# UZ-SLAMLab/DefSLAM

Measured on AMD Instinct MI355X. Metric: SfT GN iters/sec (500-node mesh, 1k matches), higher is better.
Workload: dtype f64

## Files before the change

defslam_amd/csrc/sft_batch.h:

```cpp
#pragma once

#define SFTB_NW 8
#ifndef SFTB_LIN_NW
#define SFTB_LIN_NW 8
#endif
#ifndef SFTB_LIN_WAVES
#define SFTB_LIN_WAVES 2
#endif
#ifndef SFTB_TRIAL_WAVES
#define SFTB_TRIAL_WAVES 2
#endif

__device__ __forceinline__ void sftb_ctl_lds(char* smem, Ctl*& ctl, double*& red, double*& out, double*& panel) {
  ctl = reinterpret_cast<Ctl*>(smem);
  red = reinterpret_cast<double*>(smem + 512);
  out = red + 16 * 27 + 5;
  panel = out + 32;
}

__global__ __launch_bounds__(64 * SFTB_NW, 2) void sftb_init_kernel(const SftDev* __restrict__ probs, SftRun* __restrict__ runs, int* __restrict__ counters, int* __restrict__ lin_list, int tail_below) {
  const SftDev& P = probs[blockIdx.x];
  if (blockIdx.x == 0 && threadIdx.x == 0 && (int)gridDim.x <= tail_below) counters[6] = 1;
  init_state<64 * SFTB_NW>(P);
  if (threadIdx.x == 0) {
    SftRun& R = runs[blockIdx.x];
    R.lambda = -1.0; R.ni = 2.0; R.chi_cur = 0.0; R.chi_ini = 0.0; R.rho = 0.0; R.lambda_start = 0.0;
    R.it = 0; R.qmax = 0; R.nbad = 0; R.accepted = 0; R.all_ok = 1; R.iters = 0; R.trials = 0; R.fact_ok = 1;
    R.state = P.max_iters > 0 ? SFTB_LIN : SFTB_FINISH;
    if (P.max_iters > 0) lin_list[atomicAdd(&counters[2], 1)] = blockIdx.x;
  }
}

template <int NW>
__device__ __forceinline__ void sftb_lin_problem(const SftDev& P, SftRun& R, Ctl* ctl, double* red, double* out, double* panel) {
  constexpr int NT = 64 * NW;
  const int tid = threadIdx.x;
  auto nothing = [] {};
  const double chi0 = linearise<NW, decltype(nothing), true>(P, ctl, red, out, panel, nothing);
  double lambda = R.lambda;
  if (R.it == 0) {
    double mx = 0.0;
    for (int r = tid; r < P.Dn; r += NT) mx = fmax(mx, fabs(h_diag(P, r)));
    if (tid < 6) mx = fmax(mx, fabs(P.Hcorner[tid * 8]));
    mx = block_max(mx, red);
    lambda = 1e-5 * mx;
  }
  if (tid == 0) {
    if (R.it == 0) { R.lambda = lambda; R.ni = 2.0; R.nbad = 0; }
    R.chi_cur = chi0; R.chi_ini = chi0; R.qmax = 0; R.rho = 0.0; R.accepted = 0; R.all_ok = 1; R.lambda_start = lambda;
    R.state = SFTB_TRIAL;
  }
}

__global__ __launch_bounds__(64 * SFTB_LIN_NW, SFTB_LIN_WAVES) void sftb_lin_kernel(const SftDev* __restrict__ probs, SftRun* __restrict__ runs, int* __restrict__ counters,
                                                                                  const int* __restrict__ lin_list, int B, int tail_below) {
  constexpr int NW = SFTB_LIN_NW, NT = 64 * NW;
  extern __shared__ __attribute__((aligned(16))) char smem[];
  __shared__ int next_b;
  Ctl* ctl; double *red, *out, *panel;
  sftb_ctl_lds(smem, ctl, red, out, panel);
  const int tid = threadIdx.x;
  if (counters[6] || B - counters[0] <= tail_below) {
    if (blockIdx.x == 0 && tid == 0) counters[6] = 1;
    return;
  }
  if (blockIdx.x == 0 && tid == 0) counters[7]++;
  auto fetch = [&]() { const int i = atomicAdd(&counters[3], 1); return i < counters[2] ? lin_list[i] : -1; };
  int nxt = -1;
  if (tid == 0) nxt = fetch();
  while (true) {
    if (tid == 0) next_b = nxt;
    __syncthreads();
    const int b = __builtin_amdgcn_readfirstlane(next_b);
    if (b < 0) break;
    if (tid == 0) { nxt = fetch(); atomicAdd(&counters[9], 1); }
    sftb_lin_problem<NW>(probs[b], runs[b], ctl, red, out, panel);
  }
}

__global__ __launch_bounds__(64, 1) void sftb_factor_kernel(const SftDev* __restrict__ probs, SftRun* __restrict__ runs, int* __restrict__ counters, int B) {
  extern __shared__ __attribute__((aligned(16))) char smem[];
  lds_double* lds = to_lds(reinterpret_cast<double*>(smem));
  const int lane = threadIdx.x;
  if (counters[6]) return;
  for (int i = lane; i < WV_LDS_DOUBLES; i += 64) lds[i] = 0.0;
  if (blockIdx.x == 0 && lane == 0) { counters[2] = 0; counters[3] = 0; }
  WvPrev Q;
  Q.Lg = nullptr; Q.Linv = nullptr; Q.x = nullptr; Q.nT = 0; Q.active = 0; Q.xb = 0.0;
  int n_done = 0;
  while (true) {
    int b = 0;
    if (lane == 0) b = atomicAdd(&counters[1], 1);
    b = __builtin_amdgcn_readfirstlane(b);
    if (b >= B) break;
    if (runs[b].state != SFTB_TRIAL) continue;
    const SftDev& P = probs[b];
    const double lambda = runs[b].lambda;
    double xcam;
    const int ok = wv_factor(P, lambda, lambda, lds, Q, xcam);
    if (lane == 0) runs[b].fact_ok = ok;
    Q = wv_prev_of(P, ok, xcam, lane);
    n_done++;
  }
  int lane_now;
  asm volatile("v_mbcnt_lo_u32_b32 %0, -1, 0\n\tv_mbcnt_hi_u32_b32 %0, -1, %0" : "=v"(lane_now));
  if (Q.active) wv_backsub_now(Q, lane_now);
  if (lane_now == 0 && n_done) atomicAdd(&counters[8], n_done);
}

template <int NW>
__device__ __forceinline__ int sftb_trial_problem(const SftDev& P, SftRun& R, Ctl* ctl, double* red, double* out, double* panel, int* counters, int* lin_list, int b) {
  constexpr int NT = 64 * NW;
  const int tid = threadIdx.x;
  const int Dn = P.Dn;
  const int Dnp = ((Dn + NB - 1) / NB) * NB;
  const int ok = R.fact_ok;
  const double lam = R.lambda;
  const bool in_lds = P.lds_class >= 1;
  if (!in_lds)
    for (int i = tid; i < 3 * P.n; i += NT) {
      const double v = P.xyz[i];
      P.xyz_bak[i] = v;
      const int a = P.act[i / 3];
      if (a >= 0) P.xyz[i] = v + P.x[3 * a + (i % 3)];
    }
  if (tid < 7) R.pose_bak[tid] = P.pose[tid];
  __syncthreads();
  if (tid == 0) pose_oplus(P.pose, P.x + Dnp);
  double sc = 0.0;
  for (int r = tid; r < Dn; r += NT) { const double xv = P.x[r]; sc += xv * (lam * xv + P.Hbord[(size_t)6 * Dnp + r]); }
  if (tid < 6) { const double xv = P.x[Dnp + tid]; sc += xv * (lam * xv + P.Hcorner[42 + tid]); }
  __syncthreads();
  block_sum<1>(&sc, red, out);
  const double scale = out[0];
  __syncthreads();
  const auto staged = asm_records<NW, 1>(P, panel);
  const double chi_new = in_lds ? eval_edges<false, 1>(P, ctl, red, out, staged, P.x)
                                : eval_edges<false, 0>(P, ctl, red, out, asm_records<NW, 0>(P, panel));
  if (tid == 0) {
    const double tempChi = ok ? chi_new : DBL_MAX;
    double rho = (R.chi_cur - tempChi);
    rho /= (scale + 1e-3);
    R.rho = rho;
    if (rho > 0 && isfinite(tempChi)) {
      double alpha = 1. - pow((2 * rho - 1), 3);
      alpha = fmin(alpha, 2. / 3.);
      const double sf = fmax(1. / 3., alpha);
      R.lambda = lam * sf; R.ni = 2.0; R.chi_cur = tempChi; R.accepted = 1;
      ctl->stop = 0;
    } else {
      R.lambda = lam * R.ni; R.ni *= 2.0;
      ctl->stop = 1;
    }
    R.qmax++;
    R.all_ok &= ok;
    ctl->qmax = R.qmax;
    ctl->rho = rho;
  }
  __syncthreads();
  if (ctl->stop) {
    if (!in_lds)
      for (int i = tid; i < 3 * P.n; i += NT) P.xyz[i] = P.xyz_bak[i];
    if (tid < 7) P.pose[tid] = R.pose_bak[tid];
  } else if (in_lds) {
    for (int i = tid; i < 3 * P.n; i += NT) P.xyz[i] = staged.xyz_l[i];
  }
  const bool again = (ctl->rho < 0) && (ctl->qmax < 10);
  if (again) return 0;
  __syncthreads();
  if (tid == 0) {
    const int qmax = R.qmax;
    R.trials += qmax;
    R.iters++;
    if (P.trace) {
      double* t = P.trace + R.it * 8;
      t[0] = R.chi_ini; t[1] = R.lambda_start; t[2] = qmax; t[3] = R.chi_cur; t[4] = R.lambda; t[5] = R.rho; t[6] = R.accepted; t[7] = R.all_ok;
    }
    if (!R.all_ok) P.res->status |= 1;
    bool term = (qmax == 10) || (R.rho == 0);
    if (!term) {
      if ((R.chi_ini - R.chi_cur) * 1e3 < R.chi_ini) R.nbad++; else R.nbad = 0;
      term = R.nbad >= 3;
    }
    R.it++;
    if (R.it >= P.max_iters) term = true;
    ctl->nbad = term ? 1 : 0;
    ctl->it = R.iters;
    ctl->accepted = R.trials;
    R.state = term ? SFTB_DONE : SFTB_LIN;
// ... 83 lines not shown
```

defslam_amd/csrc/sft_wave.h:

```cpp
#pragma once

#if defined(WV_STEP_TRACE) && defined(DSH_LAB)
#define WV_T_DECL long long wv_tr[9] = {0, 0, 0, 0, 0, 0, 0, 0, 0}, wv_tl = clock64()
#define WV_T(e) do { const long long t__ = clock64(); wv_tr[e] += t__ - wv_tl; wv_tl = t__; } while (0)
#define WV_T_ARG , long long (&wv_tr)[9], long long& wv_tl
#define WV_T_PASS , wv_tr, wv_tl
#define WV_T_DUMP(P) do { if ((threadIdx.x & 63) == 0) for (int e__ = 0; e__ < 9; e__++) (P).dbg[40 + e__] = (double)wv_tr[e__]; } while (0)
#else
#define WV_T_DECL do {} while (0)
#define WV_T(e) do {} while (0)
#define WV_T_ARG
#define WV_T_PASS
#define WV_T_DUMP(P) do {} while (0)
#endif

__host__ __device__ constexpr int wv_phys(int r, int d) {
  return d == 0 ? r : (d <= 3 ? 8 * d + r : (d == 4 ? 32 + (r & 3) : 8 * (8 - d) + ((r + 8 - d) & 7)));
}
constexpr int WV_AGPR_TILES = 32;
constexpr int WV_L_WIN = 0;
constexpr int WV_L_BORD = 1024;
constexpr int WV_L_WSCR = 2048;
constexpr int WV_L_CN = 2336;
constexpr int WV_L_XRING = 2400;
constexpr int WV_L_LAND = 2528;
constexpr int WV_LDS_DOUBLES = WV_L_LAND + 10 * 256;
typedef double v2d_w __attribute__((ext_vector_type(2)));
#ifndef WV_DMA_AUX
#define WV_DMA_AUX 0
#endif
using lds_v2d = __attribute__((address_space(3))) v2d_w;

#define WV_NOP_MFMA_RESULT "s_nop 15\n\ts_nop 3"

template <int T>
__device__ __forceinline__ void wv_upd_agpr(const v4d& A, const v4d& B, int q0 = 0) {
  static_assert(T >= 0 && T < WV_AGPR_TILES, "accumulator tile");
#define WV_MF(q) asm volatile("v_mfma_f64_16x16x4_f64 a[%c0:%c1], %2, %3, a[%c0:%c1] neg:[1,0,0]" ::"i"(8 * T), "i"(8 * T + 7), "v"(A[q]), "v"(B[q]) : "memory")
  if (q0 <= 0) WV_MF(0);
  if (q0 <= 1) WV_MF(1);
  if (q0 <= 2) WV_MF(2);
  WV_MF(3);
#undef WV_MF
}
__device__ __forceinline__ void wv_upd_vgpr(v4d& C, const v4d& A, const v4d& B, int q0 = 0) {
#define WV_MF(q) asm volatile("v_mfma_f64_16x16x4_f64 %0, %1, %2, %0 neg:[1,0,0]" : "+v"(C) : "v"(A[q]), "v"(B[q]) : "memory")
  asm volatile("s_nop 1" : "+v"(C));
  if (q0 <= 0) WV_MF(0);
  if (q0 <= 1) WV_MF(1);
  if (q0 <= 2) WV_MF(2);
  WV_MF(3);
#undef WV_MF
}
template <int T>
__device__ __forceinline__ void wv_trsm_agpr(v4d& Y, const v4d& Wt) {
  asm volatile("v_mfma_f64_16x16x4_f64 %0, %1, a[%c5:%c6], 0\n\t"
               "v_mfma_f64_16x16x4_f64 %0, %2, a[%c7:%c8], %0\n\t"
               "v_mfma_f64_16x16x4_f64 %0, %3, a[%c9:%c10], %0\n\t"
               "v_mfma_f64_16x16x4_f64 %0, %4, a[%c11:%c12], %0"
               : "=&v"(Y)
               : "v"(Wt[0]), "v"(Wt[1]), "v"(Wt[2]), "v"(Wt[3]), "i"(8 * T), "i"(8 * T + 1), "i"(8 * T + 2), "i"(8 * T + 3), "i"(8 * T + 4), "i"(8 * T + 5),
                 "i"(8 * T + 6), "i"(8 * T + 7)
               : "memory");
}
__device__ __forceinline__ void wv_trsm_vgpr(v4d& Y, const v4d& Wt, const v4d& D, int q0 = 0) {
  if (q0 <= 0) {
    asm volatile("s_nop 1\n\t"
                 "v_mfma_f64_16x16x4_f64 %0, %1, %5, 0\n\t"
                 "v_mfma_f64_16x16x4_f64 %0, %2, %6, %0\n\t"
                 "v_mfma_f64_16x16x4_f64 %0, %3, %7, %0\n\t"
                 "v_mfma_f64_16x16x4_f64 %0, %4, %8, %0"
                 : "=&v"(Y)
                 : "v"(Wt[0]), "v"(Wt[1]), "v"(Wt[2]), "v"(Wt[3]), "v"(D[0]), "v"(D[1]), "v"(D[2]), "v"(D[3])
                 : "memory");
  } else {
    asm volatile("s_nop 1\n\tv_mfma_f64_16x16x4_f64 %0, %1, %2, 0" : "=&v"(Y) : "v"(Wt[3]), "v"(D[3]) : "memory");
    if (q0 <= 2) asm volatile("v_mfma_f64_16x16x4_f64 %0, %1, %2, %0" : "+v"(Y) : "v"(Wt[2]), "v"(D[2]) : "memory");
    if (q0 <= 1) asm volatile("v_mfma_f64_16x16x4_f64 %0, %1, %2, %0" : "+v"(Y) : "v"(Wt[1]), "v"(D[1]) : "memory");
  }
}
struct WvTri { double a[10]; };
__device__ __forceinline__ void wv_tri_load(const lds_double* wscr, int lane, WvTri& A) {
  const lds_double* p = wscr + (lane & 3) * 17 + (lane >> 4);
#pragma unroll
  for (int q = 0; q < 4; q++)
#pragma unroll
    for (int k = 0; k <= q; k++) A.a[q * (q + 1) / 2 + k] = p[68 * q + 4 * k];
}
#define WV_TRI_BODY(D0, D1, D2, D3)                          \
  "v_mfma_f64_4x4x4_4b_f64 %3, %10, " D0 ", 0\n\t"   \
  "v_mfma_f64_4x4x4_4b_f64 %2, %7, " D0 ", 0\n\t"    \
  "v_mfma_f64_4x4x4_4b_f64 %3, %11, " D1 ", %3\n\t"  \
  "v_mfma_f64_4x4x4_4b_f64 %2, %8, " D1 ", %2\n\t"   \
  "v_mfma_f64_4x4x4_4b_f64 %3, %12, " D2 ", %3\n\t"  \
  "v_mfma_f64_4x4x4_4b_f64 %2, %9, " D2 ", %2\n\t"   \
  "v_mfma_f64_4x4x4_4b_f64 %3, %13, " D3 ", %3\n\t"  \
  "v_mfma_f64_4x4x4_4b_f64 %1, %5, " D0 ", 0\n\t"    \
  "v_mfma_f64_4x4x4_4b_f64 %0, %4, " D0 ", 0\n\t"    \
  "v_mfma_f64_4x4x4_4b_f64 %1, %6, " D1 ", %1"
template <int T>
__device__ __forceinline__ void wv_trsm4_agpr(v4d& Y, const WvTri& A) {
  asm volatile(WV_TRI_BODY("a[%c14:%c15]", "a[%c16:%c17]", "a[%c18:%c19]", "a[%c20:%c21]")
               : "=&v"(Y[0]), "=&v"(Y[1]), "=&v"(Y[2]), "=&v"(Y[3])
               : "v"(A.a[0]), "v"(A.a[1]), "v"(A.a[2]), "v"(A.a[3]), "v"(A.a[4]), "v"(A.a[5]), "v"(A.a[6]), "v"(A.a[7]), "v"(A.a[8]), "v"(A.a[9]),
                 "i"(8 * T), "i"(8 * T + 1), "i"(8 * T + 2), "i"(8 * T + 3), "i"(8 * T + 4), "i"(8 * T + 5), "i"(8 * T + 6), "i"(8 * T + 7)
               : "memory");
// ... 115 lines not shown
  w = (v4d){(g == c) ? 1.0 : 0.0, (g + 4 == c) ? 1.0 : 0.0, (g + 8 == c) ? 1.0 : 0.0, (g + 12 == c) ? 1.0 : 0.0};
  double plast = 1.0;
#pragma unroll
  for (int J = 0; J < 4; J++) {
    const double aJ = a[J];
    const double sel = chol4_inverse_operand(aJ, J, g, c & 3, plast);
    const double wJ = w[J];
    double zw, lp;
    if (J < 3) {
      asm volatile("s_nop 1\n\t"
                   "v_mfma_f64_4x4x4_4b_f64 %0, %2, %3, 0\n\t"
                   "v_mfma_f64_4x4x4_4b_f64 %1, %2, %4, 0\n\t"
                   "s_nop 7"
                   : "=&v"(zw), "=&v"(lp)
                   : "v"(sel), "v"(wJ), "v"(aJ));
      const double nlp = -lp;
      const double below = (c >= 4 * J + 4) ? nlp : 0.0;
      asm volatile("s_nop 1\n\t"
                   "v_mfma_f64_16x16x4_f64 %0, %2, %3, %0\n\t"
                   "v_mfma_f64_16x16x4_f64 %1, %4, %5, %1\n\t" WV_NOP_MFMA_RESULT
                   : "+v"(a), "+v"(w)
                   : "v"(nlp), "v"(lp), "v"(below), "v"(zw));
      w[J] = zw;
    } else {
      asm volatile("s_nop 1\n\tv_mfma_f64_4x4x4_4b_f64 %0, %1, %2, 0\n\ts_nop 7" : "=&v"(zw) : "v"(sel), "v"(wJ));
      w[J] = zw;
    }
  }
  return plast > 0.0;
}

struct WvProb {
  int Dn, Dnp, nT, q8;
  double lambda, lam_corner;
  unsigned bofs;
  const SFT_G double* Hc;
  const SFT_G uint32_t* hgl;
  const SFT_G double* Hbord;
  SFT_G double *Lg, *Linv;
};

typedef unsigned v4u_w __attribute__((ext_vector_type(4)));
__device__ __forceinline__ void wv_list(const WvProb& W, int I, int d, int lane, unsigned (&o)[4]) {
  const SFT_G v4u_w* row = reinterpret_cast<const SFT_G v4u_w*>(W.hgl + ((size_t)(I < W.nT ? I : W.nT) * (BT + 1) + d) * 256);
  const v4u_w v = row[lane];
  o[0] = v.x; o[1] = v.y; o[2] = v.z; o[3] = v.w;
}
__device__ __forceinline__ v4d wv_gather_vgpr(const WvProb& W, const unsigned (&o)[4]) {
  const auto b8 = reinterpret_cast<const SFT_G char*>(W.Hc);
  v4d v;
#pragma unroll
  for (int q = 0; q < 4; q++) v[q] = *reinterpret_cast<const SFT_G double*>(b8 + o[q]);
  return v;
}
__device__ __forceinline__ WvB2 wv_border_fresh(const WvProb& W, int J, int lane) {
  const SFT_G double* p = W.Hbord + TS * (J < W.nT ? J : W.nT);
  (void)lane;
  return WvB2{p[W.bofs], p[W.bofs + 4 * (unsigned)W.Dnp]};
}

struct WvRowList { unsigned o[8][4]; };
__device__ __forceinline__ void wv_row_list(const WvProb& W, int I, int lane, WvRowList& L) {
#pragma unroll
  for (int d = 0; d < 8; d++) wv_list(W, I, d, lane, L.o[d]);
}
template <int PH, int D>
__device__ __forceinline__ void wv_row_fetch_d(const WvProb& W, const WvRowList& L, int dmax, v4d& fresh4) {
  if constexpr (D < 8) {
    if (D <= dmax) {
      if constexpr (D == 4) fresh4 = wv_gather_vgpr(W, L.o[D]);
      else wv_gather_agpr<wv_phys(PH, D)>(W.Hc, L.o[D][0], L.o[D][1], L.o[D][2], L.o[D][3]);
    }
    wv_row_fetch_d<PH, D + 1>(W, L, dmax, fresh4);
  }
}

struct WvPrev {
  const SFT_G double* Lg;
  const SFT_G double* Linv;
  SFT_G double* x;
  int nT, active;
  double xb;
};
__device__ __forceinline__ void wv_bs_request(const WvPrev& Q, int J, lds_double* land, int lane) {
  const unsigned voff = 16u * (unsigned)lane;
  const SFT_G char* col = reinterpret_cast<const SFT_G char*>(Q.Lg + ((size_t)J * (BT + 1)) * 256);
  const SFT_G char* w = reinterpret_cast<const SFT_G char*>(Q.Linv + (size_t)J * 256);
  const unsigned l0 = (unsigned)__builtin_amdgcn_readfirstlane((int)(size_t)land);
  asm volatile("s_mov_b32 m0, %2\n\ts_nop 0\n\t"
               "global_load_lds_dwordx4 %0, %1\n\t"
               "global_load_lds_dwordx4 %0, %1 offset:2048\n\t"
               "global_load_lds_dwordx4 %0, %1 offset:3072"
               :: "v"(voff), "s"(col), "s"(l0) : "memory", "m0");
#pragma unroll
  for (int grp = 1; grp < 5; grp++) {
    const SFT_G char* cg = col + 4096 * grp;
    const unsigned lg = l0 + 4096u * grp;
    if (grp < 4)
      asm volatile("s_mov_b32 m0, %2\n\ts_nop 0\n\t"
                   "global_load_lds_dwordx4 %0, %1\n\t"
                   "global_load_lds_dwordx4 %0, %1 offset:1024\n\t"
                   "global_load_lds_dwordx4 %0, %1 offset:2048\n\t"
                   "global_load_lds_dwordx4 %0, %1 offset:3072"
                   :: "v"(voff), "s"(cg), "s"(lg) : "memory", "m0");
    else
      asm volatile("s_mov_b32 m0, %2\n\ts_nop 0\n\t"
                   "global_load_lds_dwordx4 %0, %1\n\t"
                   "global_load_lds_dwordx4 %0, %1 offset:1024"
                   :: "v"(voff), "s"(cg), "s"(lg) : "memory", "m0");
  }
  asm volatile("s_mov_b32 m0, %2\n\ts_nop 0\n\t"
               "global_load_lds_dwordx4 %0, %1\n\t"
               "global_load_lds_dwordx4 %0, %1 offset:1024"
               :: "v"(voff), "s"(w), "s"(l0 + 18u * 1024u) : "memory", "m0");
}
__device__ __forceinline__ void wv_bs_column(const WvPrev& Q, int J, const lds_double* land, lds_double* xring, int lane) {
  const int c = lane & 15;
  const lds_v2d* t2 = reinterpret_cast<const lds_v2d*>(land) + 2 * lane;
  double s[4];
  {
    const lds_double* tb = land + wv_bstd_index(lane);
    s[0] = tb[0] * Q.xb; s[1] = tb[8] * Q.xb; s[2] = tb[16] * Q.xb; s[3] = tb[24] * Q.xb;
  }
#pragma unroll
  for (int d = 1; d <= 8; d++) {
    const double xr = xring[((J + d) & 7) * 16 + c];
    const v2d_w a = t2[128 * d], b = t2[128 * d + 1];
    s[0] = fma(a.x, xr, s[0]); s[1] = fma(a.y, xr, s[1]); s[2] = fma(b.x, xr, s[2]); s[3] = fma(b.y, xr, s[3]);
  }
#pragma unroll
  for (int q = 0; q < 4; q++) {
    s[q] += wv_dpp_mov<0x128>(s[q]);
    s[q] += wv_dpp_mov<0x124>(s[q]);
    s[q] += wv_dpp_mov<0x122>(s[q]);
    s[q] += wv_dpp_mov<0x121>(s[q]);
  }
  const v2d_w wa = t2[128 * 9], wb = t2[128 * 9 + 1];
  double p = wa.x * -s[0];
  p = fma(wa.y, -s[1], p); p = fma(wb.x, -s[2], p); p = fma(wb.y, -s[3], p);
  p = sum_rows(p);
  if (lane < TS) { xring[(J & 7) * 16 + lane] = p; Q.x[TS * J + lane] = p; }
}
__device__ __forceinline__ void wv_bs_step(const WvPrev& Q, int J, lds_double* lds, int lane) {
  wv_bs_column(Q, J, lds + WV_L_LAND, lds + WV_L_XRING, lane);
  asm volatile("s_waitcnt lgkmcnt(0)" ::: "memory");
  if (J >= 1) wv_bs_request(Q, J - 1, lds + WV_L_LAND, lane);
}
__device__ __forceinline__ void wv_bs_begin(const WvPrev& Q, lds_double* lds, int lane) {
  lds_double* xring = lds + WV_L_XRING;
  xring[lane] = 0.0; xring[64 + lane] = 0.0;
  wv_bs_request(Q, Q.nT - 1, lds + WV_L_LAND, lane);
}
__device__ __forceinline__ void wv_backsub_now(const WvPrev& Q, int lane) {
  const int c = lane & 15;
  (void)c;
  double xr[8];
#pragma unroll
  for (int s = 0; s < 8; s++) xr[s] = 0.0;
  struct Col { v4d t[10]; };
  auto fetch = [&](int J) -> Col {
    Col C;
    if (J >= 0) {
      const SFT_G double* col = Q.Lg + ((size_t)J * (BT + 1)) * 256 + 4 * lane;
#pragma unroll
      for (int i = 1; i <= 8; i++) C.t[i] = (J + i < Q.nT) ? *reinterpret_cast<const SFT_G v4d*>(col + 256 * i) : (v4d){0.0, 0.0, 0.0, 0.0};
      {
        const SFT_G double* tb = col - 4 * lane + wv_bstd_index(lane);
        C.t[0] = (v4d){tb[0], tb[8], tb[16], tb[24]};
      }
      C.t[9] = *reinterpret_cast<const SFT_G v4d*>(Q.Linv + (size_t)J * 256 + 4 * lane);
    } else {
#pragma unroll
      for (int i = 0; i < 10; i++) C.t[i] = (v4d){0.0, 0.0, 0.0, 0.0};
    }
    return C;
  };
  auto solve_col = [&](const Col& C, int J, auto phc) {
    constexpr int ph = decltype(phc)::value;
    double s[4];
#pragma unroll
    for (int q = 0; q < 4; q++) s[q] = C.t[0][q] * Q.xb;
#pragma unroll
    for (int dd = 1; dd <= 8; dd++)
#pragma unroll
      for (int q = 0; q < 4; q++) s[q] = fma(C.t[dd][q], xr[(ph + dd) & 7], s[q]);
#pragma unroll
    for (int q = 0; q < 4; q++) {
      s[q] += wv_dpp_mov<0x128>(s[q]);
      s[q] += wv_dpp_mov<0x124>(s[q]);
      s[q] += wv_dpp_mov<0x122>(s[q]);
      s[q] += wv_dpp_mov<0x121>(s[q]);
    }
    double p = C.t[9][0] * -s[0];
#pragma unroll
    for (int q = 1; q < 4; q++) p = fma(C.t[9][q], -s[q], p);
    p = sum_rows(p);
    xr[ph] = p;
    if (lane < TS) Q.x[TS * J + lane] = p;
  };
  int J = Q.nT - 1;
  Col c0 = fetch(J), c1 = fetch(J - 1);
#pragma unroll 1
  for (; J >= 0; J -= 2) {
    const Col n0 = fetch(J - 2), n1 = fetch(J - 3);
    switch (J & 7) {
      case 7: solve_col(c0, J, std::integral_constant<int, 7>{}); solve_col(c1, J - 1, std::integral_constant<int, 6>{}); break;
      case 5: solve_col(c0, J, std::integral_constant<int, 5>{}); solve_col(c1, J - 1, std::integral_constant<int, 4>{}); break;
      case 3: solve_col(c0, J, std::integral_constant<int, 3>{}); solve_col(c1, J - 1, std::integral_constant<int, 2>{}); break;
      default: solve_col(c0, J, std::integral_constant<int, 1>{}); solve_col(c1, J - 1, std::integral_constant<int, 0>{}); break;
    }
    c0 = n0; c1 = n1;
  }
}

struct WvState {
  v4d Y[9];
  WvB2 Yq;
  WvBO Yo;
  double corner;
  v4d araw;
  WvB2 bnext;
  WvRowList rl;
  unsigned al[4];
  unsigned off_lane, off_bord;
  int ok;
};

template <int PH, int I, int IEND>
__device__ __forceinline__ void wv_trsm_cols(WvState& S, const WvTri& Wt, int k, int nT, const v4d& D4, int lane) {
  if constexpr (I <= IEND) {
    (void)k; (void)nT;
    if constexpr (I == 4) {
      wv_trsm4_vgpr(S.Y[4], Wt, D4);
    } else {
      wv_trsm4_agpr<wv_phys((PH + I) & 7, I)>(S.Y[I], Wt);
    }
    wv_trsm_cols<PH, I + 1, IEND>(S, Wt, k, nT, D4, lane);
  }
}

__host__ __device__ constexpr int wv_tile_index(int I, int J) {
  int n = 0;
  for (int i = 1; i <= 7; i++)
    for (int j = 1; j <= i; j++) {
      if (i == I && j == J) return n;
      if (i - j != 4) n++;
    }
  return n;
}
template <int PH, int SLOT>
__device__ __forceinline__ void wv_fetch_slot(const WvProb& W, const WvRowList& L) {
  if constexpr (SLOT < 28) {
    constexpr int t = SLOT / 4, q = SLOT % 4, d = t < 4 ? t : t + 1;
    wv_gather1_agpr<wv_phys(PH, d), q>(W.Hc, L.o[d][q]);
  }
}
template <int PH, bool TAIL, int I, int J>
__device__ __forceinline__ void wv_update_tiles(const WvProb& W, WvState& S, int k, int nT, int q8, SFT_G double* col) {
  if constexpr (I <= 8) {
    constexpr int d = I - J, r = (PH + I) & 7;
    if constexpr (d != 4) {
      if (!TAIL || k + I < nT) wv_upd_agpr<wv_phys(r, d)>(S.Y[J], S.Y[I], (I == 8) ? q8 : 0);
      if constexpr (I <= 7) {
        constexpr int n = wv_tile_index(I, J);
        if constexpr (n < 18) {
          const SFT_G double* slot = col + 256 * (n >> 1);
          if constexpr (n == 0) {
            const v2d_w yb = (v2d_w){S.Yq.n0, S.Yq.n1};
            asm volatile("global_store_dwordx4 %0, %1, %2" :: "v"(S.off_bord), "v"(yb), "s"(slot) : "memory");
          } else if constexpr (n >= 2) {
            const v4d& y = S.Y[n >> 1];
            const v2d_w half = (v2d_w){y[2 * (n & 1)], y[2 * (n & 1) + 1]};
            asm volatile("global_store_dwordx4 %0, %1, %2 offset:%c3" :: "v"(S.off_lane), "v"(half), "s"(slot), "n"(16 * (n & 1)) : "memory");
          }
        }
        wv_fetch_slot<PH, 2 * n>(W, S.rl);
        wv_fetch_slot<PH, 2 * n + 1>(W, S.rl);
      }
    }
    if constexpr (J < I) wv_update_tiles<PH, TAIL, I, J + 1>(W, S, k, nT, q8, col);
  }
}
template <int PH, bool TAIL, int I0, int I1>
__device__ __forceinline__ void wv_update_rows(const WvProb& W, WvState& S, int k, int nT, int q8, SFT_G double* col) {
  if constexpr (I0 <= I1) {
    wv_update_tiles<PH, TAIL, I0, 1>(W, S, k, nT, q8, col);
    wv_update_rows<PH, TAIL, I0 + 1, I1>(W, S, k, nT, q8, col);
  }
}
template <int PH, int T>
__device__ __forceinline__ lds_double* wv_task_tile(lds_double* lds) {
  if constexpr (T < 7) return lds + WV_L_BORD + 128 * ((PH + T + 1) & 7);
  else if constexpr (T < 10) return lds + WV_L_WIN + 256 * (wv_phys((PH + T - 2) & 7, 4) - WV_AGPR_TILES);
  else if constexpr (T == 10) return lds + WV_L_BORD + 128 * (PH & 7);
// ... 258 lines not shown
      case 14: wv_step_rest<6, true>(W, S, w, k, lds, lane, Q WV_T_PASS); break;
      default: wv_step_rest<7, true>(W, S, w, k, lds, lane, Q WV_T_PASS); break;
    }
  }
  WV_T_DUMP(P);
  if (Q.active) {
    for (int J = Q.nT - 1 - W.nT; J >= 0; J--) { wv_wait_vm(); wv_bs_step(Q, J, lds, lane); }
  }
#ifdef DSH_LAB
  const long long wv_t2 = clock64();
  const long long wv_w2 = wall_clock64();
#endif
  wv_mfma_fence();
  {
    int l2;
    asm volatile("v_mbcnt_lo_u32_b32 %0, -1, 0\n\tv_mbcnt_hi_u32_b32 %0, -1, %0" : "=v"(l2));
    const int g2 = l2 >> 4, c2 = l2 & 15;
    const int cr2 = 4 * (c2 >> 3) + g2, cc2 = 4 * ((c2 >> 2) & 1) + (c2 & 3);
    if (cr2 < SFT_BORDER && cc2 < SFT_BORDER) Cn[cr2 * 7 + cc2] = S.corner;
  }
  double xcam = 0.0;
  {
    int okc = 1;
    if (lane == 0) {
      double xc[6] = {0, 0, 0, 0, 0, 0};
      bool bad = false;
      for (int kk = 0; kk < 6; kk++) {
        double dd = Cn[kk * 7 + kk];
        for (int j = 0; j < kk; j++) dd -= Cn[kk * 7 + j] * Cn[kk * 7 + j];
        if (!(dd > 0.0)) bad = true;
        const double piv = sqrt(dd);
        Cn[kk * 7 + kk] = piv;
        for (int r = kk + 1; r < 7; r++) {
          double v = Cn[r * 7 + kk];
          for (int j = 0; j < kk; j++) v -= Cn[r * 7 + j] * Cn[kk * 7 + j];
          Cn[r * 7 + kk] = v / piv;
        }
      }
      if (bad) okc = 0;
      for (int kk = 5; kk >= 0; kk--) {
        double v = Cn[6 * 7 + kk];
        for (int r = kk + 1; r < 6; r++) v -= Cn[r * 7 + kk] * xc[r];
        xc[kk] = v / Cn[kk * 7 + kk];
      }
      for (int kk = 0; kk < 6; kk++) Cn[49 + kk] = xc[kk];
    }
    okc = __builtin_amdgcn_readfirstlane(okc);
    if (!okc) S.ok = 0;
    if (c < 6) xcam = Cn[49 + c];
  }
  xcam_out = xcam;
#ifdef DSH_LAB
  if (lane == 0) { P.dbg[5] = (double)(wv_t1 - wv_t0); P.dbg[6] = (double)(wv_t2 - wv_t1); P.dbg[4] = (double)(wv_w2 - wv_w1); }
#endif
  return __builtin_amdgcn_readfirstlane(S.ok);
}

__device__ __forceinline__ WvPrev wv_prev_of(const SftDev& P, int ok, double xcam, int lane_) {
  (void)lane_;
  int lane;
  asm volatile("v_mbcnt_lo_u32_b32 %0, -1, 0\n\tv_mbcnt_hi_u32_b32 %0, -1, %0" : "=v"(lane));
  const int c = lane & 15;
  WvPrev Q;
  const int Dn = uni(P.Dn), Dnp = ((Dn + NB - 1) / NB) * NB;
  Q.Lg = uni(P.Lb); Q.Linv = uni(P.Linv); Q.x = uni(P.x);
  Q.nT = Dnp / TS;
  Q.active = ok;
  Q.xb = (c < 6) ? xcam : ((c == 6) ? -1.0 : 0.0);
  if (ok && lane < 6) P.x[Dnp + lane] = xcam;
  return Q;
}

__device__ __forceinline__ int wv_factor_solve(const SftDev& P, double lambda, double lam_corner, lds_double* lds) {
  WvPrev none;
  none.Lg = nullptr; none.Linv = nullptr; none.x = nullptr; none.nT = 0; none.active = 0; none.xb = 0.0;
  double xcam;
  const int ok = wv_factor(P, lambda, lam_corner, lds, none, xcam);
  int lane;
  asm volatile("v_mbcnt_lo_u32_b32 %0, -1, 0\n\tv_mbcnt_hi_u32_b32 %0, -1, %0" : "=v"(lane));
  const WvPrev Q = wv_prev_of(P, ok, xcam, lane);
#ifdef DSH_LAB
  const long long t2 = clock64();
#endif
  if (ok) wv_backsub_now(Q, lane);
#ifdef DSH_LAB
  if (lane == 0) P.dbg[7] = (double)(clock64() - t2);
#endif
  return ok;
}
```

Measured before the change: 417,700.

## Restructure wave back-substitution around LDS landing layout with split-reduction and staged prefetch

Reworks the banded block back-substitution so each lane-group handles a distinct row subset, reading tiles from a remapped LDS landing buffer instead of holding per-lane v4d columns and doing four DPP reductions per column. Global-to-LDS DMA requests are now issued per kilobyte with a padded two-half layout and split into two parts that interleave with the column's reduction tail. The register-resident backsub path now stages fetched columns through LDS and reuses the same column kernel. This aims to cut cross-lane reduction work and register pressure on the serial solve, at the cost of extra LDS traffic and round trips per column.

New measurement: 419,700 (median of 6 runs). About the same (+0.5%).

```diff
diff --git a/defslam_amd/csrc/sft_batch.h b/defslam_amd/csrc/sft_batch.h
--- a/defslam_amd/csrc/sft_batch.h
+++ b/defslam_amd/csrc/sft_batch.h
@@ -104,7 +104,7 @@
   }
   int lane_now;
   asm volatile("v_mbcnt_lo_u32_b32 %0, -1, 0\n\tv_mbcnt_hi_u32_b32 %0, -1, %0" : "=v"(lane_now));
-  if (Q.active) wv_backsub_now(Q, lane_now);
+  if (Q.active) wv_backsub_now(Q, lds, lane_now);
   if (lane_now == 0 && n_done) atomicAdd(&counters[8], n_done);
 }
 
diff --git a/defslam_amd/csrc/sft_wave.h b/defslam_amd/csrc/sft_wave.h
--- a/defslam_amd/csrc/sft_wave.h
+++ b/defslam_amd/csrc/sft_wave.h
@@ -21,7 +21,9 @@
 constexpr int WV_L_WIN = 0;
 constexpr int WV_L_BORD = 1024;
 constexpr int WV_L_WSCR = 2048;
+constexpr int WV_L_STURN = 2320;
 constexpr int WV_L_CN = 2336;
+constexpr int WV_L_XB = 2392;
 constexpr int WV_L_XRING = 2400;
 constexpr int WV_L_LAND = 2528;
 constexpr int WV_LDS_DOUBLES = WV_L_LAND + 10 * 256;
@@ -303,134 +305,143 @@
   int nT, active;
   double xb;
 };
+constexpr int WV_LAND_PITCH = 1024;
+constexpr int WV_LAND_HALF2 = 8 * 1024 + 128;
+static_assert(2047 + WV_LAND_HALF2 + 9 * WV_LAND_PITCH < 10 * 2048, "landing buffer");
+__device__ __forceinline__ unsigned wv_land_map(unsigned o) { return o < 1024u ? o : o + (unsigned)WV_LAND_HALF2; }
+using lds_char = __attribute__((address_space(3))) char;
+constexpr int WV_BS_AHEAD = 4;
+
+template <int GOFF, int LOFF>
+__device__ __forceinline__ void wv_bs_request_kb(unsigned voff, const SFT_G char* col, unsigned l0) {
+  constexpr int imm = GOFF % 4096;
+  asm volatile("s_add_u32 m0, %2, %c3\n\ts_nop 0\n\t"
+               "global_load_lds_dwordx4 %0, %1 offset:%c4"
+               :: "v"(voff), "s"(col + (GOFF - imm)), "s"(l0), "n"(LOFF - imm), "n"(imm) : "memory", "m0", "scc");
+}
+template <int I>
+__device__ __forceinline__ void wv_bs_request_tiles(unsigned voff, const SFT_G char* col, unsigned l0) {
+  if constexpr (I <= 8) {
+    wv_bs_request_kb<2048 * I, WV_LAND_PITCH * I>(voff, col, l0);
+    wv_bs_request_kb<2048 * I + 1024, 1024 + WV_LAND_HALF2 + WV_LAND_PITCH * I>(voff, col, l0);
+    wv_bs_request_tiles<I + 1>(voff, col, l0);
+  }
+}
+template <int PART = 0>
 __device__ __forceinline__ void wv_bs_request(const WvPrev& Q, int J, lds_double* land, int lane) {
   const unsigned voff = 16u * (unsigned)lane;
-  const SFT_G char* col = reinterpret_cast<const SFT_G char*>(Q.Lg + ((size_t)J * (BT + 1)) * 256);
-  const SFT_G char* w = reinterpret_cast<const SFT_G char*>(Q.Linv + (size_t)J * 256);
   const unsigned l0 = (unsigned)__builtin_amdgcn_readfirstlane((int)(size_t)land);
-  asm volatile("s_mov_b32 m0, %2\n\ts_nop 0\n\t"
-               "global_load_lds_dwordx4 %0, %1\n\t"
-               "global_load_lds_dwordx4 %0, %1 offset:2048\n\t"
-               "global_load_lds_dwordx4 %0, %1 offset:3072"
-               :: "v"(voff), "s"(col), "s"(l0) : "memory", "m0");
-#pragma unroll
-  for (int grp = 1; grp < 5; grp++) {
-    const SFT_G char* cg = col + 4096 * grp;
-    const unsigned lg = l0 + 4096u * grp;
-    if (grp < 4)
-      asm volatile("s_mov_b32 m0, %2\n\ts_nop 0\n\t"
-                   "global_load_lds_dwordx4 %0, %1\n\t"
-                   "global_load_lds_dwordx4 %0, %1 offset:1024\n\t"
-                   "global_load_lds_dwordx4 %0, %1 offset:2048\n\t"
-                   "global_load_lds_dwordx4 %0, %1 offset:3072"
-                   :: "v"(voff), "s"(cg), "s"(lg) : "memory", "m0");
-    else
-      asm volatile("s_mov_b32 m0, %2\n\ts_nop 0\n\t"
-                   "global_load_lds_dwordx4 %0, %1\n\t"
-                   "global_load_lds_dwordx4 %0, %1 offset:1024"
-                   :: "v"(voff), "s"(cg), "s"(lg) : "memory", "m0");
-  }
-  asm volatile("s_mov_b32 m0, %2\n\ts_nop 0\n\t"
-               "global_load_lds_dwordx4 %0, %1\n\t"
-               "global_load_lds_dwordx4 %0, %1 offset:1024"
-               :: "v"(voff), "s"(w), "s"(l0 + 18u * 1024u) : "memory", "m0");
-}
-__device__ __forceinline__ void wv_bs_column(const WvPrev& Q, int J, const lds_double* land, lds_double* xring, int lane) {
-  const int c = lane & 15;
-  const lds_v2d* t2 = reinterpret_cast<const lds_v2d*>(land) + 2 * lane;
-  double s[4];
+  if constexpr (PART != 2) {
+    const SFT_G char* col = reinterpret_cast<const SFT_G char*>(Q.Lg + ((size_t)J * (BT + 1)) * 256);
+    wv_bs_request_kb<0, 0>(voff, col, l0);
+    wv_bs_request_tiles<1>(voff, col, l0);
+  }
+  if constexpr (PART != 1) {
+    const SFT_G char* w = reinterpret_cast<const SFT_G char*>(Q.Linv + (size_t)J * 256);
+    wv_bs_request_kb<0, WV_LAND_PITCH * 9>(voff, w, l0);
+    wv_bs_request_kb<1024, 1024 + WV_LAND_HALF2 + WV_LAND_PITCH * 9>(voff, w, l0);
+  }
+}
+template <bool REQ = false>
+__device__ __forceinline__ void wv_bs_column(const WvPrev& Q, int J, lds_double* lds, int lane) {
+  const int g = lane >> 4, c = lane & 15;
+  const lds_char* land = reinterpret_cast<const lds_char*>(lds + WV_L_LAND);
+  lds_double* xring = lds + WV_L_XRING;
+  lds_double* turn = lds + WV_L_STURN;
+  const lds_char* el = land + wv_land_map(512u * (c & 3) + 32u * g + 8u * (c >> 2));
+  double a[4];
   {
-    const lds_double* tb = land + wv_bstd_index(lane);
-    s[0] = tb[0] * Q.xb; s[1] = tb[8] * Q.xb; s[2] = tb[16] * Q.xb; s[3] = tb[24] * Q.xb;
-  }
+    const v2d_w yb = *reinterpret_cast<const lds_v2d*>(land + 16 * (16 * (c & 3) + 4 * (c >> 2) + g));
+    const v2d_w xb = *reinterpret_cast<const lds_v2d*>(lds + WV_L_XB + 2 * g);
+    a[0] = yb.x * xb.x; a[1] = yb.y * xb.y;
+  }
+  struct Tile { v2d_w x01, x23; double e[4]; };
+  auto load = [&](int d) -> Tile {
+    Tile T;
+    const lds_v2d* xr = reinterpret_cast<const lds_v2d*>(xring + ((J + d) & 7) * 16 + 4 * g);
+    T.x01 = xr[0]; T.x23 = xr[1];
+    const lds_char* t = el + WV_LAND_PITCH * d;
+#pragma unroll
+    for (int q = 0; q < 4; q++) T.e[q] = *reinterpret_cast<const volatile lds_double*>(t + 128 * q);
+    return T;
+  };
+  Tile T[9];
+#pragma unroll
+  for (int d = 1; d <= WV_BS_AHEAD; d++) T[d] = load(d);
 #pragma unroll
   for (int d = 1; d <= 8; d++) {
-    const double xr = xring[((J + d) & 7) * 16 + c];
-    const v2d_w a = t2[128 * d], b = t2[128 * d + 1];
-    s[0] = fma(a.x, xr, s[0]); s[1] = fma(a.y, xr, s[1]); s[2] = fma(b.x, xr, s[2]); s[3] = fma(b.y, xr, s[3]);
-  }
-#pragma unroll
-  for (int q = 0; q < 4; q++) {
-    s[q] += wv_dpp_mov<0x128>(s[q]);
-    s[q] += wv_dpp_mov<0x124>(s[q]);
-    s[q] += wv_dpp_mov<0x122>(s[q]);
-    s[q] += wv_dpp_mov<0x121>(s[q]);
-  }
-  const v2d_w wa = t2[128 * 9], wb = t2[128 * 9 + 1];
-  double p = wa.x * -s[0];
-  p = fma(wa.y, -s[1], p); p = fma(wb.x, -s[2], p); p = fma(wb.y, -s[3], p);
+    if (d + WV_BS_AHEAD <= 8) T[d + WV_BS_AHEAD] = load(d + WV_BS_AHEAD);
+    __builtin_amdgcn_sched_barrier(0);
+    a[0] = fma(T[d].e[0], T[d].x01.x, a[0]); a[1] = fma(T[d].e[1], T[d].x01.y, a[1]);
+    if (d == 1) { a[2] = T[d].e[2] * T[d].x23.x; a[3] = T[d].e[3] * T[d].x23.y; }
+    else { a[2] = fma(T[d].e[2], T[d].x23.x, a[2]); a[3] = fma(T[d].e[3], T[d].x23.y, a[3]); }
+    __builtin_amdgcn_sched_barrier(0);
+  }
+  double s = sum_rows((a[0] + a[1]) + (a[2] + a[3]));
+  const lds_v2d* wt = reinterpret_cast<const lds_v2d*>(land + wv_land_map(32u * lane) + WV_LAND_PITCH * 9);
+  const v2d_w wa = wt[0], wb = wt[1];
+  turn[4 * (c & 3) + (c >> 2)] = s;
+  const lds_v2d* sp = reinterpret_cast<const lds_v2d*>(turn + 4 * g);
+  const v2d_w s01 = sp[0], s23 = sp[1];
+  if (REQ && J >= 1) {
+    asm volatile("" : "+v"(s));
+    wv_bs_request<1>(Q, J - 1, lds + WV_L_LAND, lane);
+  }
+  double p = wa.x * -s01.x;
+  p = fma(wa.y, -s01.y, p); p = fma(wb.x, -s23.x, p); p = fma(wb.y, -s23.y, p);
+  if (REQ && J >= 1) {
+    asm volatile("" : "+v"(p));
+    wv_bs_request<2>(Q, J - 1, lds + WV_L_LAND, lane);
+  }
   p = sum_rows(p);
-  if (lane < TS) { xring[(J & 7) * 16 + lane] = p; Q.x[TS * J + lane] = p; }
-}
-__device__ __forceinline__ void wv_bs_step(const WvPrev& Q, int J, lds_double* lds, int lane) {
-  wv_bs_column(Q, J, lds + WV_L_LAND, lds + WV_L_XRING, lane);
-  asm volatile("s_waitcnt lgkmcnt(0)" ::: "memory");
-  if (J >= 1) wv_bs_request(Q, J - 1, lds + WV_L_LAND, lane);
-}
-__device__ __forceinline__ void wv_bs_begin(const WvPrev& Q, lds_double* lds, int lane) {
+  if (lane < TS) { xring[(J & 7) * 16 + 4 * (lane & 3) + (lane >> 2)] = p; Q.x[TS * J + lane] = p; }
+}
+__device__ __forceinline__ void wv_bs_step(const WvPrev& Q, int J, lds_double* lds, int lane) { wv_bs_column<true>(Q, J, lds, lane); }
+__device__ __forceinline__ void wv_bs_init(const WvPrev& Q, lds_double* lds, int lane) {
   lds_double* xring = lds + WV_L_XRING;
   xring[lane] = 0.0; xring[64 + lane] = 0.0;
+  if (lane < 8) lds[WV_L_XB + 2 * (lane & 3) + (lane >> 2)] = Q.xb;
+}
+__device__ __forceinline__ void wv_bs_begin(const WvPrev& Q, lds_double* lds, int lane) {
+  wv_bs_init(Q, lds, lane);
   wv_bs_request(Q, Q.nT - 1, lds + WV_L_LAND, lane);
 }
-__device__ __forceinline__ void wv_backsub_now(const WvPrev& Q, int lane) {
-  const int c = lane & 15;
-  (void)c;
-  double xr[8];
-#pragma unroll
-  for (int s = 0; s < 8; s++) xr[s] = 0.0;
-  struct Col { v4d t[10]; };
+__device__ __forceinline__ void wv_backsub_now(const WvPrev& Q, lds_double* lds, int lane) {
+  struct Col { v4d t[10]; v2d_w yb; };
   auto fetch = [&](int J) -> Col {
     Col C;
     if (J >= 0) {
-      const SFT_G double* col = Q.Lg + ((size_t)J * (BT + 1)) * 256 + 4 * lane;
-#pragma unroll
-      for (int i = 1; i <= 8; i++) C.t[i] = (J + i < Q.nT) ? *reinterpret_cast<const SFT_G v4d*>(col + 256 * i) : (v4d){0.0, 0.0, 0.0, 0.0};
-      {
-        const SFT_G double* tb = col - 4 * lane + wv_bstd_index(lane);
-        C.t[0] = (v4d){tb[0], tb[8], tb[16], tb[24]};
-      }
+      const SFT_G double* col = Q.Lg + ((size_t)J * (BT + 1)) * 256;
+#pragma unroll
+      for (int i = 1; i <= 8; i++) C.t[i] = (J + i < Q.nT) ? *reinterpret_cast<const SFT_G v4d*>(col + 256 * i + 4 * lane) : (v4d){0.0, 0.0, 0.0, 0.0};
+      C.yb = *reinterpret_cast<const SFT_G v2d_w*>(col + 2 * lane);
       C.t[9] = *reinterpret_cast<const SFT_G v4d*>(Q.Linv + (size_t)J * 256 + 4 * lane);
     } else {
 #pragma unroll
-      for (int i = 0; i < 10; i++) C.t[i] = (v4d){0.0, 0.0, 0.0, 0.0};
+      for (int i = 1; i < 10; i++) C.t[i] = (v4d){0.0, 0.0, 0.0, 0.0};
+      C.yb = (v2d_w){0.0, 0.0};
     }
     return C;
   };
-  auto solve_col = [&](const Col& C, int J, auto phc) {
-    constexpr int ph = decltype(phc)::value;
-    double s[4];
-#pragma unroll
-    for (int q = 0; q < 4; q++) s[q] = C.t[0][q] * Q.xb;
-#pragma unroll
-    for (int dd = 1; dd <= 8; dd++)
-#pragma unroll
-      for (int q = 0; q < 4; q++) s[q] = fma(C.t[dd][q], xr[(ph + dd) & 7], s[q]);
-#pragma unroll
-    for (int q = 0; q < 4; q++) {
-      s[q] += wv_dpp_mov<0x128>(s[q]);
-      s[q] += wv_dpp_mov<0x124>(s[q]);
-      s[q] += wv_dpp_mov<0x122>(s[q]);
-      s[q] += wv_dpp_mov<0x121>(s[q]);
-    }
-    double p = C.t[9][0] * -s[0];
-#pragma unroll
-    for (int q = 1; q < 4; q++) p = fma(C.t[9][q], -s[q], p);
-    p = sum_rows(p);
-    xr[ph] = p;
-    if (lane < TS) Q.x[TS * J + lane] = p;
+  lds_char* land = reinterpret_cast<lds_char*>(lds + WV_L_LAND);
+  auto land_col = [&](const Col& C) {
+    *reinterpret_cast<lds_v2d*>(land + 16 * lane) = C.yb;
+    lds_v2d* own = reinterpret_cast<lds_v2d*>(land + wv_land_map(32u * lane));
+#pragma unroll
+    for (int i = 1; i <= 9; i++) {
+      own[(WV_LAND_PITCH / 16) * i] = (v2d_w){C.t[i][0], C.t[i][1]};
+      own[(WV_LAND_PITCH / 16) * i + 1] = (v2d_w){C.t[i][2], C.t[i][3]};
+    }
   };
+  wv_bs_init(Q, lds, lane);
   int J = Q.nT - 1;
   Col c0 = fetch(J), c1 = fetch(J - 1);
 #pragma unroll 1
-  for (; J >= 0; J -= 2) {
-    const Col n0 = fetch(J - 2), n1 = fetch(J - 3);
-    switch (J & 7) {
-      case 7: solve_col(c0, J, std::integral_constant<int, 7>{}); solve_col(c1, J - 1, std::integral_constant<int, 6>{}); break;
-      case 5: solve_col(c0, J, std::integral_constant<int, 5>{}); solve_col(c1, J - 1, std::integral_constant<int, 4>{}); break;
-      case 3: solve_col(c0, J, std::integral_constant<int, 3>{}); solve_col(c1, J - 1, std::integral_constant<int, 2>{}); break;
-      default: solve_col(c0, J, std::integral_constant<int, 1>{}); solve_col(c1, J - 1, std::integral_constant<int, 0>{}); break;
-    }
-    c0 = n0; c1 = n1;
+  for (; J >= 0; J--) {
+    const Col n = fetch(J - 2);
+    land_col(c0);
+    wv_bs_column(Q, J, lds, lane);
+    c0 = c1; c1 = n;
   }
 }
 
@@ -855,7 +866,7 @@
 #ifdef DSH_LAB
   const long long t2 = clock64();
 #endif
-  if (ok) wv_backsub_now(Q, lane);
+  if (ok) wv_backsub_now(Q, lds, lane);
 #ifdef DSH_LAB
   if (lane == 0) P.dbg[7] = (double)(clock64() - t2);
 #endif
```
